# yehonatan145/PatternMatching

Hardware: AMD Instinct MI355X
Metric: GB/s stream scanned + matches/sec, snort.dict, 1/2/4/8 MI355X vs CPU ref (higher is better)
Workload: dtype u8

## Files before the change

### patternmatching_amd/csrc/pm_kernels.hip

```cpp
#include <type_traits>

#include <algorithm>

#include "pm_kernels.h"
#include "pm_streamgen.h"

namespace {

#ifdef RT_PLAIN_STORES
#define RT_OUT_STORE(v, p) (*(p) = (v))
#else
#define RT_OUT_STORE(v, p) __builtin_nontemporal_store((v), (p))
#endif
constexpr int RT_THREADS = 1024;
constexpr int RT_WAVES = RT_THREADS / 64;
constexpr int RT_T2_U16 = 65536;
constexpr int RT_FILTER_WORDS = 4096;
constexpr int RT_F3_WORDS = 256;
constexpr int RT_F2_WORDS = 2048;
constexpr uint32_t RT_QCAP = 64;
constexpr uint32_t RT_ROUND = 40;
constexpr int RT_CHUNK = 1024;
constexpr uint32_t CONT16 = 0x8000u;
constexpr uint32_t CONT32 = 0x80000000u;
constexpr uint32_t T3H_VALID = 1u << 24;
constexpr uint32_t RT_POSMASK = (1u << 30) - 1;
constexpr uint32_t RT_SLOT2 = 1u << 30;
constexpr uint32_t RT_REC_LEAF_K = 0, RT_REC_KIDS_K = 1, RT_REC_CHAIN_K = 2, RT_REC_WIDE_K = 3;

__device__ __forceinline__ uint32_t rt_hash(uint32_t k) { return k * 0x9E3779B1u; }
__device__ __forceinline__ uint32_t rt_fhash(uint32_t k) {
    uint32_t h;
    asm("v_mul_u32_u24 %0, 0x9e3779, %1" : "=v"(h) : "v"(k));
    return h;
}
__device__ __forceinline__ uint32_t rt_fhit(uint32_t w, uint32_t f) {
    uint32_t a, b, c;
    asm("v_lshrrev_b32_e32 %0, %1, %2" : "=v"(a) : "v"(f), "v"(w));
    asm("v_lshrrev_b32_sdwa %0, %1, %2 dst_sel:DWORD dst_unused:UNUSED_PAD src0_sel:BYTE_1 src1_sel:DWORD"
        : "=v"(b) : "v"(f), "v"(w));
    asm("v_lshrrev_b32_sdwa %0, %1, %2 dst_sel:DWORD dst_unused:UNUSED_PAD src0_sel:BYTE_2 src1_sel:DWORD"
        : "=v"(c) : "v"(f), "v"(w));
    return a & b & c & 1u;
}

struct Stage2 {
    uint32_t g3, g4, w3, w4;
};
__device__ __forceinline__ Stage2 rt_stage2_load(const uint32_t* s_f2, uint32_t q) {
    Stage2 z;
    asm("v_mul_u32_u24 %0, 0x85ebca, %1" : "=v"(z.g3) : "v"(q >> 8));
    z.g4 = q * 0x9E3779B1u;
    z.w3 = s_f2[z.g3 >> 24];
    z.w4 = s_f2[RT_F3_WORDS + (((z.g4 >> 20) * 7u) >> 4)];
    return z;
}
__device__ __forceinline__ uint32_t rt_stage2_hit(const Stage2& z) { return rt_fhit(z.w3, z.g3) | rt_fhit(z.w4, z.g4); }

__device__ __forceinline__ uint32_t wave_scan_incl(uint32_t x) {
    x += __builtin_amdgcn_update_dpp(0u, x, 0x111, 0xf, 0xf, false);
    x += __builtin_amdgcn_update_dpp(0u, x, 0x112, 0xf, 0xf, false);
    x += __builtin_amdgcn_update_dpp(0u, x, 0x114, 0xf, 0xf, false);
    x += __builtin_amdgcn_update_dpp(0u, x, 0x118, 0xf, 0xf, false);
    x += __builtin_amdgcn_update_dpp(0u, x, 0x142, 0xa, 0xf, false);
    x += __builtin_amdgcn_update_dpp(0u, x, 0x143, 0xc, 0xf, false);
    return x;
}

__device__ __forceinline__ uint32_t wave_prefix(uint64_t m) {
    return __builtin_amdgcn_mbcnt_hi((uint32_t)(m >> 32), __builtin_amdgcn_mbcnt_lo((uint32_t)m, 0u));
}

template <class V4>
__device__ __forceinline__ uint32_t rec_kind(const V4& R) { return R.x >> 30; }
template <class V4>
__device__ __forceinline__ uint32_t rec_kid_index(const V4& R, uint32_t c) {
    const uint32_t c4 = c * 0x01010101u;
    const uint32_t lo = R.z ^ c4, hi = R.w ^ c4;
    const uint32_t zl = (lo - 0x01010101u) & ~lo & 0x80808080u;
    const uint32_t zh = (hi - 0x01010101u) & ~hi & 0x80808080u;
    const uint32_t cnt = (R.x >> 24) & 63u;
    const uint32_t j = zl ? (uint32_t)__builtin_ctz(zl) >> 3 : zh ? 4u + ((uint32_t)__builtin_ctz(zh) >> 3) : 8u;
    return j < cnt ? j : cnt;
}

template <class V4>
__device__ __forceinline__ uint32_t wide_child(const V4& Q, uint32_t c) {
    const uint32_t odd = (c >> 5) & 1u, bit = c & 31u;
    const uint32_t word = odd ? Q.y : Q.x;
    if (!((word >> bit) & 1u)) return ~0u;
    return Q.z + (odd ? (uint32_t)__popc(Q.x) : 0u) + (uint32_t)__popc(word & ((1u << bit) - 1u));
}

template <bool FOLD>
__device__ __forceinline__ uint32_t rt_byte(const uint8_t* __restrict__ text, int64_t k) {
    uint32_t c = text[k];
    if (FOLD) c += c - 'A' < 26u ? 32u : 0u;
    return c;
}

template <bool FOLD = false>
__device__ __forceinline__ uint32_t rt_deep(const uint8_t* __restrict__ text, const RtDev& t, uint32_t node, int64_t i,
                                            int64_t avail, int64_t d) {
    for (;;) {
        const uint4 R = t.rec[node];
        if (d >= avail) return R.y;
        const uint32_t c = rt_byte<FOLD>(text, i - d);
        const uint32_t kind = rec_kind(R), first = R.x & 0xFFFFFFu;
        if (kind == RT_REC_LEAF_K) return R.y;
        if (kind == RT_REC_CHAIN_K) {
            const uint32_t L = (R.x >> 24) & 63u;
            const uint32_t lim = avail - d < (int64_t)L ? (uint32_t)(avail - d) : L;
            uint64_t win = 0;
#pragma unroll
            for (int k = 0; k < 8; ++k) {
                const uint32_t kk = (uint32_t)k < lim ? (uint32_t)k : lim - 1u;
                win |= (uint64_t)rt_byte<FOLD>(text, i - d - kk) << (8 * (7 - k));
            }
            const uint64_t dif = win ^ ((uint64_t)R.w << 32 | R.z);
            uint32_t m = dif ? (uint32_t)__builtin_clzll(dif) >> 3 : 8u;
            m = m < lim ? m : lim;
            if (m < L) return R.y;
            node = first + m - 1u;
            d += m;
            continue;
        } else if (kind == RT_REC_KIDS_K) {
            const uint32_t j = rec_kid_index(R, c);
            if (j == ((R.x >> 24) & 63u)) return R.y;
            node = first + j;
        } else {
            const uint32_t ch = wide_child(t.wide[(size_t)R.z * 4 + (c >> 6)], c);
            if (ch == ~0u) return R.y;
            node = ch;
        }
        ++d;
    }
}

__device__ __forceinline__ uint32_t rt_slot1(uint32_t k, uint32_t bits) { return rt_hash(k) >> (32 - bits); }
__device__ __forceinline__ uint32_t rt_slot2(uint32_t k, uint32_t bits) { return (k * 0x85EBCA77u) >> (32 - bits); }

template <bool FOLD = false>
__device__ __forceinline__ uint32_t rt_from_d2(const uint8_t* __restrict__ text, const RtDev& t, uint32_t key24,
                                               uint32_t c3, uint32_t best2, int64_t i, int64_t avail) {
    const uint32_t want = T3H_VALID | key24;
    uint4 e = t.t3h[rt_slot1(key24, t.t3h_bits)];
    if ((e.x & 0x1FFFFFFu) != want) {
        e = t.t3h[rt_slot2(key24, t.t3h_bits)];
        if ((e.x & 0x1FFFFFFu) != want) return best2;
    }
    const uint32_t kind = e.x >> 25;
    if (kind == 0 || avail < 4) return e.y;
    if (kind == 1) {
        const uint32_t nch = e.z >> 24;
        const uint32_t k = c3 == (e.z & 0xFFu) ? 0u : c3 == ((e.z >> 8) & 0xFFu) ? 1u : c3 == ((e.z >> 16) & 0xFFu) ? 2u : 3u;
        if (k >= nch) return e.y;
        if (nch > 1) return rt_deep<FOLD>(text, t, e.w + k, i, avail, 4);
        if (!(e.w & CONT32)) return e.w;
        return rt_deep<FOLD>(text, t, e.w & 0x7FFFFFFFu, i, avail, 4);
    }
    return rt_deep<FOLD>(text, t, e.w & 0x7FFFFFFFu, i, avail, 3);
}

template <bool FOLD = false>
__device__ uint32_t rt_one(const uint8_t* __restrict__ text, const uint16_t* s_t, const RtDev& t, int64_t i,
                           int64_t stream_start) {
    const int64_t avail = i - stream_start + 1;
    const uint32_t c0 = rt_byte<FOLD>(text, i);
    if (avail == 1) return t.t12[65536 + c0];
    const uint32_t c1 = rt_byte<FOLD>(text, i - 1);
    const uint32_t v = s_t[(c0 << 8) | c1];
    if (!(v & CONT16) || avail == 2) return v & 0x7FFFu;
    return rt_from_d2<FOLD>(text, t, rt_byte<FOLD>(text, i - 2) | (c1 << 8) | (c0 << 16),
                            avail >= 4 ? rt_byte<FOLD>(text, i - 3) : 0u, v & 0x7FFFu, i, avail);
}
// ... 118 lines not shown
            const uint64_t m = __ballot(need);
            const uint32_t idx = nxt + wave_prefix(m);
            if (need && idx < nwalk) {
                z.st = TS_ENTRY;
                z.c = idx & 1u;
                z.pa = reinterpret_cast<const tu32x4*>(items + (idx & ~1u));
                z.pb = dummy2;
            }
            nxt += (uint32_t)__popcll(m);
            if (nxt > nwalk) nxt = nwalk;
            busy |= z.st != TS_EMPTY;
        });
        if (!__ballot(busy)) break;
        unroll_for<0, SLOTS>([&](auto I) __attribute__((always_inline)) {
            TailSlot& z = S[I];
            z.A = *z.pa;
            z.B = *z.pb;
        });
        unroll_for<0, SLOTS>([&](auto I) __attribute__((always_inline)) {
            TailSlot& z = S[I];
            const uint32_t st = z.st;
            const tu32x4 A = z.A;
            const uint32_t en = z.c ? A.z : A.x, ep = z.c ? A.w : A.y;
            const uint32_t off = z.pos & RT_POSMASK;
            const int32_t rq = (int32_t)off - (int32_t)z.dd;
            const bool reload = rq < z.twa || rq >= z.twa + 8;
            const uint32_t rlo = reload ? z.B.x : z.tlo, rhi = reload ? z.B.y : z.thi;
            const int32_t rta = reload ? (rq & ~7) : z.twa;
            const uint32_t ro = (uint32_t)(rq - rta);
            const uint32_t c = ((ro & 4 ? rhi : rlo) >> (8 * (ro & 3))) & 0xFFu;
            const uint32_t rkind = rec_kind(A), first = A.x & 0xFFFFFFu;
            const uint32_t jr = rec_kid_index(A, c);
            const bool rend = z.dd >= z.av;
            const bool rnext = !rend && rkind == RT_REC_KIDS_K && jr != ((A.x >> 24) & 63u);
            const bool rwide = !rend && rkind == RT_REC_WIDE_K;
            const uint64_t win = ((uint64_t)rhi << 32 | rlo) << (8 * (7 - ro));
            const uint64_t dif = win ^ ((uint64_t)A.w << 32 | A.z);
            const uint32_t meq = dif ? (uint32_t)__builtin_clzll(dif) >> 3 : 8u;
            const uint32_t clen = (A.x >> 24) & 63u;
            const uint32_t cav = z.av > z.dd ? z.av - z.dd : 0u;
            const uint32_t clim = min(min(clen, ro + 1u), cav);
            const uint32_t cm = min(meq, clim);
            const bool cnext = rkind == RT_REC_CHAIN_K && cm >= 1u && (cm == clen || (cm == ro + 1u && cm < cav));
            const uint32_t wnode = wide_child(A, z.c);
            const bool wnext = wnode != ~0u;

            uint32_t nst = TS_EMPTY;
            bool fin = false;
            uint32_t ans = A.w;
            if (st == TS_ENTRY) {
                nst = TS_REC;
                z.node = en;
                z.dd = (ep & RT_D4) ? 4u : 3u;
                z.pos = ep & ~RT_D4;
                const uint32_t o = ep & RT_POSMASK;
                z.av = o + ctx + 1 > 1024u ? 1024u : o + ctx + 1;
                z.twa = INT32_MIN / 2;
            }
            if (st == TS_REC) {
                nst = (rnext || cnext) ? TS_REC : rwide ? TS_WIDE : TS_EMPTY;
                fin = !rnext && !rwide && !cnext;
                ans = A.y;
                z.tlo = rlo;
                z.thi = rhi;
                z.twa = rta;
                z.node = cnext ? first + cm - 1u : first + jr;
                z.dd += rnext ? 1u : cnext ? cm : 0u;
                z.c = c;
            }
            if (st == TS_WIDE) {
                nst = wnext ? TS_REC : TS_EMPTY;
                fin = !wnext;
                z.node = wnode;
                z.dd += 1;
            }
            if (fin) {
                cnt += (uint32_t)(ans != 0u) - (z.pos >> 31);
                if (OUTW) put_id<OUTW>(out, (int64_t)(z.pos & RT_POSMASK), ans);
            }
            z.st = nst;
            const int32_t nq = (int32_t)(z.pos & RT_POSMASK) - (int32_t)z.dd;
            const bool nreload = z.dd < z.av && (nq < z.twa || nq >= z.twa + 8);
            const tu32x4* pa = dummy4;
            const tu32x2* pb = dummy2;
            if (nst == TS_REC) {
                pa = RC + z.node;
                if (nreload) pb = reinterpret_cast<const tu32x2*>(tb + (nq & ~7));
            }
            if (nst == TS_WIDE) pa = WD + (size_t)A.z * 4 + (c >> 6);
            z.pa = pa;
            z.pb = pb;
        });
    }
    return nwalk;
}

template <int V, int OUTW, bool EF = false>
__global__ __launch_bounds__(RT_THREADS) void rt_scan_kernel(const uint8_t* __restrict__ text, int64_t stream_start,
                                                             int64_t pos0, int64_t n, void* __restrict__ out,
                                                             unsigned long long* __restrict__ count, RtDev t) {
    static_assert(V == 0 || V == 2, "product kernel (0) or streaming floor (2)");
    constexpr bool kT8 = V == 0 && OUTW == 0;
    constexpr int kLdsWords = kT8 ? RT_T2_U16 / 4 + RT_F2_WORDS + 2 * RT_WAVES * RT_QCAP
                                  : RT_FILTER_WORDS + RT_T2_U16 / 2 + RT_F2_WORDS + 2 * RT_WAVES * RT_QCAP;
    __shared__ __attribute__((aligned(16))) uint32_t s_lds[kLdsWords];
    uint32_t* const s_f = s_lds;
    const uint8_t* const s_t8 = reinterpret_cast<const uint8_t*>(s_lds);
    const uint16_t* const s_t = kT8 ? t.t12 : reinterpret_cast<uint16_t*>(s_lds + RT_FILTER_WORDS);
    uint32_t* const s_f2 = s_lds + (kT8 ? RT_T2_U16 / 4 : RT_FILTER_WORDS + RT_T2_U16 / 2);
    uint32_t(*const s_qkey)[RT_QCAP] = reinterpret_cast<uint32_t(*)[RT_QCAP]>(s_f2 + RT_F2_WORDS);
    uint32_t(*const s_qpos)[RT_QCAP] = s_qkey + RT_WAVES;
    {
        const uint4* fsrc = reinterpret_cast<const uint4*>(t.filt);
        if (kT8) {
            const uint2* src = reinterpret_cast<const uint2*>(t.t12);
            for (int k = threadIdx.x; k < RT_T2_U16 / 4; k += RT_THREADS) {
                const uint2 v = src[k];
                const uint32_t e[4] = {v.x & 0xFFFFu, v.x >> 16, v.y & 0xFFFFu, v.y >> 16};
                uint32_t w = 0;
#pragma unroll
                for (int q = 0; q < 4; ++q) {
                    const uint32_t nz = (e[q] & 0x7FFFu) != 0u, cand = !nz && (e[q] & CONT16);
                    w |= (nz | cand << 1) << (8 * q);
                }
                s_lds[k] = w;
            }
        } else {
            const uint4* src = reinterpret_cast<const uint4*>(t.t12);
            uint4* dst = reinterpret_cast<uint4*>(s_lds + RT_FILTER_WORDS);
            for (int k = threadIdx.x; k < RT_T2_U16 * 2 / 16; k += RT_THREADS) dst[k] = src[k];
            uint4* fdst = reinterpret_cast<uint4*>(s_f);
            for (int k = threadIdx.x; k < RT_FILTER_WORDS / 4; k += RT_THREADS) fdst[k] = fsrc[k];
        }
        uint4* f2dst = reinterpret_cast<uint4*>(s_f2);
        for (int k = threadIdx.x; k < RT_F2_WORDS / 4; k += RT_THREADS) f2dst[k] = fsrc[RT_FILTER_WORDS / 4 + k];
    }
    __syncthreads();

    constexpr bool kFilter = V == 0;
    constexpr bool kPushS2 = V == 0 && OUTW == 4;
    constexpr bool kRounds = !(V == 0 && OUTW == 0);
    constexpr bool kStage1 = !(V == 0 && OUTW == 0);
    const int lane = threadIdx.x & 63;
    const int wid = __builtin_amdgcn_readfirstlane(threadIdx.x >> 6);
    uint32_t* qkey = s_qkey[wid];
    uint32_t* qpos = s_qpos[wid];
    uint32_t cnt = 0;
    uint32_t scnt = 0;
    const int64_t nchunks = (n + RT_CHUNK - 1) / RT_CHUNK;
    const int64_t c_hi = n / RT_CHUNK;
    const int64_t c_lo = pos0 - stream_start >= 2 ? 0 : 1;
    const int64_t gw = (int64_t)blockIdx.x * RT_WAVES + wid;
    const int64_t nw = (int64_t)gridDim.x * RT_WAVES;
    const int64_t cbeg = c_lo + gw, cend = c_hi, cstep = nw;
    uint32_t* const sp = t.spill + 2 * gw * t.spill_stride;
    uint32_t sn = 0;
    const uint8_t* dummy = reinterpret_cast<const uint8_t*>(t.filt) + 4;
    using u32x2 = __attribute__((ext_vector_type(2))) unsigned int;
    using u32x4 = __attribute__((ext_vector_type(4))) unsigned int;

    struct Round {
        uint32_t n;
        uint32_t keep;
        uint32_t fk, fp;
        u32x2 tw;
        uint32_t skip;
        u32x4 L0;
    };
    uint32_t qh = 0, qn = 0;
    auto issue = [&](Round& r, uint32_t take) __attribute__((always_inline)) {
        __builtin_amdgcn_wave_barrier();
        const bool act = (uint32_t)lane < take;
        const uint32_t sl = (qh + lane) & (RT_QCAP - 1);
        r.fk = act ? qkey[sl] : 0u;
        r.fp = act ? qpos[sl] : 0u;
        const bool deep = r.fp >> 31;
        bool skip = false;
        if (!kPushS2 && take) {
            const bool first = act && !deep && !(r.fp & RT_SLOT2);
            if (first) skip = rt_stage2_hit(rt_stage2_load(s_f2, r.fk)) == 0u;
        }
        r.skip = skip;
        r.keep = (uint32_t)__popcll(__ballot(act && !skip));
        const uint32_t k = r.fk >> 8;
        const uint32_t node = r.fk & 0x7FFFFFu, d = r.fk >> 23;
        const bool wide = deep && (r.fp & RT_SLOT2);
        const int64_t i = pos0 + (int64_t)(r.fp & RT_POSMASK);
        const u32x4* T = reinterpret_cast<const u32x4*>(t.t3h);
        const u32x4* F = reinterpret_cast<const u32x4*>(t.filt);
        const uint32_t slot = (r.fp & RT_SLOT2) ? rt_slot2(k, t.t3h_bits) : rt_slot1(k, t.t3h_bits);
        const u32x4* W = reinterpret_cast<const u32x4*>(t.wide) + (size_t)(r.fk & 0x3FFFu) * 4 + ((r.fk >> 20) & 3u);
        const u32x4* a0 = wide ? W : deep ? reinterpret_cast<const u32x4*>(t.rec) + node : ((act && !skip) ? T + slot : F);
        const uint8_t* a1 = (deep && !wide && (int64_t)d <= i - stream_start) ? text + ((i - d) & ~(int64_t)7) : dummy;
        r.L0 = *a0;
        r.tw = *reinterpret_cast<const u32x2*>(a1);
        r.n = take;
        qh += take;
        qn -= take;
    };
    auto consume = [&](Round& r) __attribute__((always_inline)) {
        u32x4 L0 = r.L0;
        u32x2 tw = r.tw;
        uint32_t fk = r.fk, fp = r.fp;
        asm volatile("" : "+v"(L0), "+v"(tw), "+v"(fk), "+v"(fp)::"memory");
        bool again = false, wstep = false;
        uint32_t nk = 0, np = 0;
        if ((uint32_t)lane < r.n && !r.skip) {
            const int64_t i = pos0 + (int64_t)(fp & RT_POSMASK);
            const int64_t avail = i - stream_start + 1;
            uint32_t v, ph0 = 0xFFFFFFFFu, node = 0, d = 0;
            bool reprobe = false;
            if (!(fp >> 31)) {
                const uint32_t k = fk >> 8, c3 = fk & 0xFFu;
                ph0 = s_t[k >> 8] & 0x7FFFu;
                const uint32_t want = T3H_VALID | k;
                const u32x4 e = L0;
                v = ph0;
                if ((e.x & 0x1FFFFFFu) != want && (e.x & T3H_VALID) && !(fp & RT_SLOT2)) {
                    reprobe = true;
                    again = true;
                } else if ((e.x & 0x1FFFFFFu) == want) {
                    v = e.y;
                    const uint32_t kind = e.x >> 25;
                    if (avail >= 4 && kind == 1) {
                        const uint32_t nch = e.z >> 24;
                        const uint32_t j = c3 == (e.z & 0xFFu) ? 0u : c3 == ((e.z >> 8) & 0xFFu) ? 1u
                                         : c3 == ((e.z >> 16) & 0xFFu) ? 2u : 3u;
                        if (j < nch) {
                            if (nch == 1 && !(e.w & CONT32)) {
                                v = e.w;
                            } else {
                                again = true;
                                node = nch == 1 ? e.w & 0x7FFFFFFFu : e.w + j;
                                d = 4;
                            }
                        }
                    } else if (avail >= 4 && kind == 2) {
                        again = true;
                        node = e.w & 0x7FFFFFFFu;
                        d = 3;
                    }
                }
            } else if (fp & RT_SLOT2) {
                const uint32_t ch = wide_child(L0, (fk >> 14) & 0xFFu);
                d = (fk >> 22) + 1;
                v = L0.w;
                if (ch != ~0u) {
                    node = ch;
                    again = true;
                }
            } else {
                d = fk >> 23;
                const u32x4 R = L0;
                v = R.y;
                if ((int64_t)d < avail) {
                    const uint32_t kind = rec_kind(R);
                    const uint32_t ro = (uint32_t)(i - d) & 7u;
                    const uint32_t tc = (((ro & 4) ? tw.y : tw.x) >> (8 * (ro & 3))) & 0xFFu;
                    if (kind == RT_REC_CHAIN_K) {
                        const uint64_t win = ((uint64_t)tw.y << 32 | tw.x) << (8 * (7 - ro));
                        const uint64_t dif = win ^ ((uint64_t)R.w << 32 | R.z);
                        const uint32_t meq = dif ? (uint32_t)__builtin_clzll(dif) >> 3 : 8u;
                        const uint32_t clen = (R.x >> 24) & 63u;
                        const uint32_t cav = (uint32_t)(avail - d);
                        const uint32_t cm = min(meq, min(min(clen, ro + 1u), cav));
                        if (cm >= 1u && (cm == clen || (cm == ro + 1u && cm < cav))) {
                            node = (R.x & 0xFFFFFFu) + cm - 1u;
                            d += cm;
                            again = true;
                        }
                    } else if (kind == RT_REC_KIDS_K) {
                        const uint32_t j = rec_kid_index(R, tc);
                        if (j != ((R.x >> 24) & 63u)) {
                            node = (R.x & 0xFFFFFFu) + j;
                            ++d;
                            again = true;
                        }
                    } else if (kind == RT_REC_WIDE_K) {
                        wstep = true;
                        again = true;
                        node = R.z | (tc << 14);
                    }
                }
            }
            if (reprobe) {
                nk = fk;
                np = fp | RT_SLOT2;
            } else if (wstep) {
                nk = node | (d << 22);
                np = fp | RT_SLOT2;
            } else if (again) {
                nk = node | (d << 23);
                np = (fp & ~RT_SLOT2) | 0x80000000u;
                if (!(fp >> 31)) cnt -= (uint32_t)(ph0 != 0u);
            } else {
                cnt += (uint32_t)(v != 0u) - ((fp >> 31) ? 0u : (uint32_t)(ph0 != 0u));
                if (OUTW && v != ph0) put_id<OUTW>(out, i - pos0, v);
            }
        }
        __builtin_amdgcn_wave_barrier();
        const uint64_t m = __ballot(again);
        if (again) {
            const uint32_t sl = (qh + qn + wave_prefix(m)) & (RT_QCAP - 1);
            qkey[sl] = nk;
            qpos[sl] = np;
        }
        __builtin_amdgcn_wave_barrier();
        qn += (uint32_t)__popcll(m);
        r.n = 0;
        r.keep = 0;
    };
    auto fetch = [&](uint32_t (&xr)[4], uint32_t& xp, int64_t c) __attribute__((always_inline)) {
        const uint8_t* base = c < cend ? text + pos0 + c * RT_CHUNK : dummy;
#pragma unroll
        for (int s = 0; s < 4; ++s)
            xr[s] = __builtin_nontemporal_load(reinterpret_cast<const uint32_t*>(base + 256 * s + 4 * lane));
        xp = __builtin_nontemporal_load(reinterpret_cast<const uint32_t*>(base - 4));
    };
    auto stand_in_store = [&]() __attribute__((always_inline)) {
        if (OUTW == 4) {
            u32x4* o = reinterpret_cast<u32x4*>(t.scratch);
#pragma unroll
            for (int s = 0; s < 4; ++s) __builtin_nontemporal_store(u32x4{0u, 0u, 0u, 0u}, o + 64 * s + lane);
        }
        if (OUTW == 2) {
            u32x2* o = reinterpret_cast<u32x2*>(t.scratch);
#pragma unroll
            for (int s = 0; s < 4; ++s) __builtin_nontemporal_store(u32x2{0u, 0u}, o + 64 * s + lane);
        }
    };
    Round rr;
    rr.n = 0;
    rr.keep = 0;
    uint32_t xa[4], xb[4], pa, pb;
    int64_t ch = cbeg;
    const uint32_t scap = (uint32_t)t.spill_stride;
    auto resolve = [&]() __attribute__((always_inline)) {
        if (!kFilter) return;
        if (rr.n) consume(rr);
        while (qn) {
            Round rs;
            issue(rs, qn);
            consume(rs);
        }
        if (kRounds && t.spill_total && sn && lane == 0) atomicAdd(t.spill_total, (unsigned long long)sn);
        __builtin_amdgcn_s_waitcnt(0);
        {
            const uint32_t nwalk = rt_tail<OUTW>(text, stream_start, pos0, out, t, s_f2, sp, sn, lane, cnt);
            if (!kRounds && t.spill_total && nwalk && lane == 0)
                atomicAdd(t.spill_total, (unsigned long long)nwalk);
        }
        __builtin_amdgcn_s_waitcnt(0);
        sn = 0;
    };
    auto chunk = [&](uint32_t (&xr)[4], uint32_t& xp, int64_t c) __attribute__((always_inline)) {
        const int64_t pc = pos0 + c * RT_CHUNK;
        u32x2 x[4];
#pragma unroll
        for (int s = 0; s < 4; ++s) {
            const uint32_t fix = s == 0 ? xp : __builtin_amdgcn_update_dpp(0u, xr[s - 1], 0x13C, 0xf, 0xf, false);
            x[s].x = __builtin_amdgcn_update_dpp(fix, xr[s], 0x138, 0xf, 0xf, false);
            x[s].y = xr[s];
        }
        if (EF) fetch(xr, xp, c + 2 * cstep);
#define RT_RAW(j) ((uint32_t)((((uint64_t)x[(j) >> 2].y << 32) | x[(j) >> 2].x) >> (8 * (2 + ((j) & 3)))))
#define RT_KEY(j) (RT_RAW(j) & 0xFFFFFFu)
        uint32_t res[16];
        constexpr int CMS = kT8 ? 1 : 0;
        uint32_t cm = 0;
        if (kT8) {
            uint32_t f = 0;
            constexpr uint32_t kSel0 = 0x0C0C0000u;
#define RT_T8KEY(j) \
    __builtin_amdgcn_perm(x[(j) >> 2].y, x[(j) >> 2].x, kSel0 | (4u + ((j) & 3)) << 8 | (3u + ((j) & 3)))
#pragma unroll
            for (int j = 0; j < 16; ++j) f |= (uint32_t)s_t8[RT_T8KEY(j)] << (2 * j);
#undef RT_T8KEY
            cnt += (uint32_t)__popc(f & 0x55555555u);
            cm = f & 0xAAAAAAAAu;
        } else {
#pragma unroll
        for (int j = 0; j < 16; ++j) res[j] = V == 2 ? RT_KEY(j) & 0xFFFFu : s_t[RT_KEY(j) >> 8];
        if (kFilter && kStage1) {
            uint32_t fw[16];
#pragma unroll
            for (int j = 0; j < 16; ++j) fw[j] = s_f[rt_fhash(RT_RAW(j)) >> 20];
#pragma unroll
            for (int j = 0; j < 16; ++j) cm |= ((res[j] >> 15) & rt_fhit(fw[j], rt_fhash(RT_RAW(j)))) << j;
        } else if (kFilter) {
#pragma unroll
            for (int j = 0; j < 16; ++j) cm |= (res[j] >> 15) << j;
        }
        if (kFilter) {
            if (OUTW == 0) {
                uint32_t zm = 0;
#pragma unroll
                for (int j = 0; j < 16; ++j) zm |= (uint32_t)((res[j] & 0x7FFFu) == 0u) << j;
                cm &= zm;
            }
        }
#pragma unroll
        for (int j = 0; j < 16; ++j) {
            res[j] &= 0x7FFFu;
            scnt += (uint32_t)__popcll(__ballot(res[j] != 0u));
        }
        }
#undef RT_KEY
#undef RT_RAW
        if (kFilter && kRounds) {
            if (rr.n) consume(rr);
            issue(rr, qn >= RT_ROUND ? qn : 0u);
        }
        if (OUTW == 4) {
            u32x4* o = reinterpret_cast<u32x4*>(reinterpret_cast<uint32_t*>(out) + (pc - pos0));
#pragma unroll
            for (int s = 0; s < 4; ++s) {
                u32x4 v = {res[4 * s], res[4 * s + 1], res[4 * s + 2], res[4 * s + 3]};
                RT_OUT_STORE(v, o + 64 * s + lane);
            }
        }
        if (OUTW == 2) {
            u32x2* o = reinterpret_cast<u32x2*>(reinterpret_cast<uint16_t*>(out) + (pc - pos0));
#pragma unroll
            for (int s = 0; s < 4; ++s) {
                u32x2 v = {res[4 * s] | (res[4 * s + 1] << 16), res[4 * s + 2] | (res[4 * s + 3] << 16)};
                RT_OUT_STORE(v, o + 64 * s + lane);
            }
        }
        asm volatile("" ::: "memory");
        if (kPushS2) {
            uint32_t mm = cm, keep = 0;
            while (mm) {
                const uint32_t bit = __builtin_ctz(mm), j = bit >> CMS;
                mm &= mm - 1;
                const uint32_t sg = j >> 2, b = j & 3;
                const u32x2 w01 = (sg & 1) ? x[1] : x[0], w23 = (sg & 1) ? x[3] : x[2];
                const u32x2 w = (sg & 2) ? w23 : w01;
                const uint32_t q32 = (uint32_t)((((uint64_t)w.y << 32) | w.x) >> (8 * (1 + b)));
                keep |= (rt_stage2_hit(rt_stage2_load(s_f2, q32)) != 0u) << bit;
            }
            cm = keep;
        }
        if (kFilter) {
            const uint32_t c = __popc(cm);
            const uint32_t incl = wave_scan_incl(c);
            const uint32_t base = incl - c;
            const uint32_t total = __builtin_amdgcn_readlane(incl, 63);
            uint32_t mm = cm;
            const uint32_t pbase = (uint32_t)(pc - pos0) + 4 * lane;
            if (kRounds && total <= RT_QCAP - qn - rr.keep) {
                uint32_t slot = qh + qn + base;
                while (mm) {
                    const uint32_t j = __builtin_ctz(mm) >> CMS;
                    mm &= mm - 1;
                    const uint32_t sg = j >> 2, b = j & 3;
                    const u32x2 w01 = (sg & 1) ? x[1] : x[0], w23 = (sg & 1) ? x[3] : x[2];
                    const u32x2 w = (sg & 2) ? w23 : w01;
                    const uint32_t sl = slot & (RT_QCAP - 1);
                    qkey[sl] = (uint32_t)((((uint64_t)w.y << 32) | w.x) >> (8 * (1 + b)));
                    qpos[sl] = pbase + 256 * sg + b;
                    ++slot;
                }
                qn += total;
            } else {
                uint32_t room = kRounds ? RT_QCAP - qn - rr.keep : 0u;
                if (__builtin_expect(sn + (total - room) > scap, 0)) {
                    resolve();
                    room = kRounds ? min(RT_QCAP, total) : 0u;
                }
                uint32_t rank = base;
                while (mm) {
                    const uint32_t j = __builtin_ctz(mm) >> CMS;
                    mm &= mm - 1;
                    const uint32_t sg = j >> 2, b = j & 3;
                    const u32x2 w01 = (sg & 1) ? x[1] : x[0], w23 = (sg & 1) ? x[3] : x[2];
                    const u32x2 w = (sg & 2) ? w23 : w01;
                    const uint32_t q32 = (uint32_t)((((uint64_t)w.y << 32) | w.x) >> (8 * (1 + b)));
                    const uint32_t p = pbase + 256 * sg + b;
                    if (rank < room) {
                        const uint32_t sl = (qh + qn + rank) & (RT_QCAP - 1);
                        qkey[sl] = q32;
                        qpos[sl] = p;
                    } else {
                        const uint32_t ph = OUTW == 0 ? 0u : (uint32_t)((s_t[q32 >> 16] & 0x7FFFu) != 0u);
                        reinterpret_cast<u32x2*>(sp)[sn + rank - room] = u32x2{q32, p | (ph << 31)};
                    }
                    ++rank;
                }
                sn = __builtin_amdgcn_readfirstlane(sn + total - room);
                qn = __builtin_amdgcn_readfirstlane(qn + room);
            }
        }
        if (!EF) fetch(xr, xp, c + 2 * cstep);
    };
    Round r0;
    if (EF) fetch(xa, pa, ch);
    if (kFilter && kRounds) issue(r0, 0);
    stand_in_store();
    if (!EF) fetch(xa, pa, ch);
    if (EF) fetch(xb, pb, ch + cstep);
    if (kFilter && kRounds) issue(rr, 0);
    stand_in_store();
    if (!EF) fetch(xb, pb, ch + cstep);
    for (;;) {
        if (ch >= cend) break;
        chunk(xa, pa, ch);
        if (ch + cstep >= cend) break;
        chunk(xb, pb, ch + cstep);
        ch += 2 * cstep;
    }
    resolve();
    if (blockIdx.x == gridDim.x - 1) {
#pragma unroll 1
        for (int e = 0; e < 2; ++e) {
            int64_t c = -1;
            if (e == 0 && c_lo == 1) c = 0;
            if (e == 1 && c_hi < nchunks && !(c_lo == 1 && c_hi == 0)) c = c_hi;
            const int64_t p = pos0 + c * RT_CHUNK + threadIdx.x;
            if (c >= 0 && p < pos0 + n) {
                const uint32_t v = rt_one(text, s_t, t, p, stream_start);
                if (OUTW) put_id<OUTW>(out, p - pos0, v);
                cnt += v != 0u;
            }
        }
    }
    if (count) {
        for (int o = 32; o > 0; o >>= 1) cnt += __shfl_down(cnt, o);
        cnt += scnt;
        if (lane == 0 && cnt) atomicAdd(count, (unsigned long long)cnt);
    }
}

constexpr int RT_SMALL_THREADS = 256;
template <int OUTW>
__global__ __launch_bounds__(RT_SMALL_THREADS) void rt_small_kernel(const uint8_t* __restrict__ text,
                                                                    int64_t stream_start, int64_t pos0, int64_t n,
                                                                    void* __restrict__ out,
                                                                    unsigned long long* __restrict__ count, RtDev t) {
    const int64_t k = (int64_t)blockIdx.x * RT_SMALL_THREADS + threadIdx.x;
    uint32_t v = 0, deep = 0;
    if (k < n) {
        const int64_t i = pos0 + k;
        v = rt_one(text, t.t12, t, i, stream_start);
        if (t.spill_total && i - stream_start >= 3 && (t.t12[(uint32_t)text[i] << 8 | text[i - 1]] & CONT16)) {
            const uint32_t q = (uint32_t)text[i - 3] | (uint32_t)text[i - 2] << 8 | (uint32_t)text[i - 1] << 16 |
                               (uint32_t)text[i] << 24;
            const uint32_t f = rt_fhash(q >> 8);
            if (rt_fhit(t.filt[f >> 20], f)) deep = rt_stage2_hit(rt_stage2_load(t.filt + RT_FILTER_WORDS, q));
        }
        if (OUTW) put_id<OUTW>(out, k, v);
    }
    const uint64_t nz = __ballot(v != 0u), dp = __ballot(deep != 0u);
    if ((threadIdx.x & 63) == 0) {
        if (count && nz) atomicAdd(count, (unsigned long long)__popcll(nz));
        if (t.spill_total && dp) atomicAdd(t.spill_total, (unsigned long long)__popcll(dp));
    }
}

constexpr int RT_SERVE_WIN = 16384;
constexpr int RT_SERVE_POLLERS = 4;
#ifndef PM_SERVE_TRACE
#define PM_SERVE_TRACE 0
#endif
__device__ __forceinline__ uint64_t rfl64(uint64_t x) {
    const uint32_t lo = __builtin_amdgcn_readfirstlane((uint32_t)x);
    const uint32_t hi = __builtin_amdgcn_readfirstlane((uint32_t)(x >> 32));
    return (uint64_t)hi << 32 | lo;
}
__device__ __forceinline__ uint64_t lane64(uint64_t x, int l) {
    const uint32_t lo = __builtin_amdgcn_readlane((uint32_t)x, l);
    const uint32_t hi = __builtin_amdgcn_readlane((uint32_t)(x >> 32), l);
    return (uint64_t)hi << 32 | lo;
}
template <class T>
__device__ __forceinline__ T sys_load(const T* p) {
    return __hip_atomic_load(p, __ATOMIC_RELAXED, __HIP_MEMORY_SCOPE_SYSTEM);
}
template <class T>
__device__ __forceinline__ void sys_store(T* p, T v) {
    __hip_atomic_store(p, v, __ATOMIC_RELAXED, __HIP_MEMORY_SCOPE_SYSTEM);
}
template <class T>
__device__ __forceinline__ T dev_load(const T* p) {
    return __hip_atomic_load(p, __ATOMIC_RELAXED, __HIP_MEMORY_SCOPE_AGENT);
}
template <class T>
__device__ __forceinline__ void dev_store(T* p, T v) {
    __hip_atomic_store(p, v, __ATOMIC_RELAXED, __HIP_MEMORY_SCOPE_AGENT);
}
__global__ __launch_bounds__(RT_SERVE_THREADS) void rt_serve_kernel(PmServeReq* req, uint64_t* fwd, uint32_t* done,
                                                                    uint64_t seen, uint64_t gen, int64_t idle_ticks,
                                                                    RtDev t) {
    __shared__ __attribute__((aligned(16))) uint8_t win[RT_SERVE_WIN];
    __shared__ uint64_t s_w[8];
    __shared__ uint32_t s_state;
    const uint64_t* const rq = reinterpret_cast<const uint64_t*>(req);
    const int tid = threadIdx.x;
    const int wid = __builtin_amdgcn_readfirstlane(tid >> 6);
    const int64_t G = gridDim.x, wg = blockIdx.x;
    if (tid == 0) s_state = 0;
    __syncthreads();
    for (;;) {
        if (wg == 0 ? wid < RT_SERVE_POLLERS : wid == 0) {
            for (int q = 0; q < wid; ++q) __builtin_amdgcn_s_sleep(24);
            const uint64_t t0 = __builtin_amdgcn_s_memrealtime();
            uint64_t w = 0;
            uint32_t found = 0, quit = 0;
            const uint64_t* const src = wg == 0 ? rq : fwd;
            for (;;) {
                w = wg == 0 ? sys_load(src + (tid & 7)) : dev_load(src + (tid & 7));
                const uint64_t s2 = lane64(w, 7);
                if (s2 > seen && s2 == lane64(w, 0)) {
                    found = 1;
                    break;
                }
                if (lane64(w, 1) == gen || __builtin_amdgcn_s_memrealtime() - t0 > (uint64_t)idle_ticks) {
                    quit = 1;
                    break;
                }
                if (wg == 0 && __builtin_amdgcn_readfirstlane(
                                   __hip_atomic_load(&s_state, __ATOMIC_RELAXED, __HIP_MEMORY_SCOPE_WORKGROUP)))
                    break;
                __builtin_amdgcn_s_sleep(1);
            }
#if PM_SERVE_TRACE
            if ((tid & 63) == 0 && wg < 2 && found)
                sys_store(reinterpret_cast<uint64_t*>(done + G + 16) + 8 * wg, __builtin_amdgcn_s_memrealtime());
#endif
            if (found) {
                const int lane = tid & 63;
                uint32_t old = 1;
                if (lane == 0) old = __hip_atomic_exchange(&s_state, 1u, __ATOMIC_RELAXED, __HIP_MEMORY_SCOPE_WORKGROUP);
                if (__builtin_amdgcn_readfirstlane(old) != 1) {
                    if (lane < 8 && lane != 1) s_w[lane] = w;
                    if (wg == 0) {
                        if (lane >= 2 && lane < 7) dev_store(fwd + lane, w);
                        __builtin_amdgcn_s_waitcnt(0);
                        if (lane == 0 || lane == 7) dev_store(fwd + lane, w);
                    }
                }
            } else if (quit && (tid & 63) == 0) {
                uint32_t zero = 0;
                __hip_atomic_compare_exchange_strong(&s_state, &zero, 2u, __ATOMIC_RELAXED, __ATOMIC_RELAXED,
                                                     __HIP_MEMORY_SCOPE_WORKGROUP);
            }
        }
        __syncthreads();
        if (__builtin_amdgcn_readfirstlane(s_state) == 2) {
            if (wg == 0 && tid == 1) dev_store(fwd + 1, gen);
            return;
        }
        __syncthreads();
        if (tid == 0) s_state = 0;
        const uint64_t v = rfl64(s_w[0]);
        seen = v;
        const uint8_t* const text = reinterpret_cast<const uint8_t*>(rfl64(s_w[2]));
        void* const out = reinterpret_cast<void*>(rfl64(s_w[3]));
        const int64_t ss = (int64_t)rfl64(s_w[4]), pos0 = (int64_t)rfl64(s_w[5]);
        const uint64_t nw = rfl64(s_w[6]);
        const int64_t n = (int64_t)(nw & ((1ull << 56) - 1));
        const bool w4 = (nw >> 56) == 4;
        const int64_t per = ((n + G - 1) / G + 63) & ~(int64_t)63;
// ... 2462 lines not shown
        for (int off = 32; off > 0; off >>= 1) cnt += __shfl_down(cnt, off);
        if ((threadIdx.x & 63) == 0 && cnt) atomicAdd(count, (unsigned long long)cnt);
    }
}

__global__ __launch_bounds__(1024) void gather_probe_kernel(const uint32_t* __restrict__ tab, uint32_t words,
                                                            int steps, uint32_t* __restrict__ sink) {
    const uint32_t lane = blockIdx.x * 1024u + threadIdx.x;
    uint32_t idx = __umulhi(lane * 0x9E3779B1u, words), acc = 0;
    for (int j = 0; j < steps; ++j) {
        const uint32_t v = tab[idx];
        acc += v;
        idx = __umulhi((v ^ (lane + (uint32_t)j)) * 0x9E3779B1u, words);
    }
    if (acc == 0x9E3779B1u && idx == 1u) sink[0] = acc;
}

__device__ __forceinline__ void score_one(uint32_t a, uint32_t r, const uint32_t* __restrict__ parent,
                                          const uint32_t* __restrict__ depth, uint32_t (&c)[5]) {
    if (a == r) {
        ++c[0];
    } else if (a) {
        uint32_t cur = r;
        while (cur && cur != a) cur = parent[cur];
        ++c[cur ? 1 : 3];
    } else {
        ++c[2];
    }
    if (r) c[4] += depth[r];
}

constexpr int SCORE_THREADS = 256;

constexpr int SCORE_V = 2;
template <int V>
__global__ __launch_bounds__(SCORE_THREADS) void score_kernel(const uint32_t* __restrict__ algo,
                                                              const uint32_t* __restrict__ real, int64_t n,
                                                              const uint32_t* __restrict__ parent,
                                                              const uint32_t* __restrict__ depth,
                                                              unsigned long long* __restrict__ counts) {
    uint32_t c[5] = {0, 0, 0, 0, 0};
    const int64_t nv = n / 4;
    const int64_t stride = (int64_t)gridDim.x * SCORE_THREADS;
    using v4 = __attribute__((ext_vector_type(4))) unsigned int;
    const v4* A = reinterpret_cast<const v4*>(algo);
    const v4* R = reinterpret_cast<const v4*>(real);
    for (int64_t k = (int64_t)blockIdx.x * SCORE_THREADS + threadIdx.x; k < nv; k += V * stride) {
        v4 a[V], r[V];
#pragma unroll
        for (int j = 0; j < V; ++j) {
            const int64_t kj = k + j * stride;
            a[j] = kj < nv ? __builtin_nontemporal_load(A + kj) : v4{0, 0, 0, 0};
            r[j] = kj < nv ? __builtin_nontemporal_load(R + kj) : v4{0, 0, 0, 0};
        }
#pragma unroll
        for (int j = 0; j < V; ++j) {
            if (k + j * stride >= nv) break;
            score_one(a[j].x, r[j].x, parent, depth, c);
            score_one(a[j].y, r[j].y, parent, depth, c);
            score_one(a[j].z, r[j].z, parent, depth, c);
            score_one(a[j].w, r[j].w, parent, depth, c);
        }
    }
    if (blockIdx.x == 0 && threadIdx.x < (n & 3)) score_one(algo[4 * nv + threadIdx.x], real[4 * nv + threadIdx.x], parent, depth, c);
#pragma unroll
    for (int q = 0; q < 5; ++q) {
        unsigned long long v = c[q];
        for (int o = 32; o > 0; o >>= 1) v += __shfl_down(v, o);
        if ((threadIdx.x & 63) == 0 && v) atomicAdd(counts + q, v);
    }
}

constexpr int HIST_THREADS = 1024;
constexpr uint32_t HIST_WINDOW = 38912;
constexpr int HIST_V = 4;

template <int V>
__global__ __launch_bounds__(HIST_THREADS) void hist_kernel(const uint32_t* __restrict__ real, int64_t n,
                                                            const uint32_t* __restrict__ parent, uint32_t lo,
                                                            uint32_t cnt, unsigned long long* __restrict__ hist) {
    __shared__ uint32_t s_h[HIST_WINDOW];
    for (uint32_t k = threadIdx.x; k < cnt; k += HIST_THREADS) s_h[k] = 0;
    __syncthreads();
    using v4 = __attribute__((ext_vector_type(4))) unsigned int;
    const int64_t nv = n / 4;
    const int64_t stride = (int64_t)gridDim.x * HIST_THREADS;
    for (int64_t k = (int64_t)blockIdx.x * HIST_THREADS + threadIdx.x; k < nv; k += V * stride) {
        uint32_t g[4 * V];
#pragma unroll
        for (int j = 0; j < V; ++j) {
            const int64_t kj = k + j * stride;
            const v4 r = kj < nv ? __builtin_nontemporal_load(reinterpret_cast<const v4*>(real) + kj) : v4{0, 0, 0, 0};
            g[4 * j] = r.x;
            g[4 * j + 1] = r.y;
            g[4 * j + 2] = r.z;
            g[4 * j + 3] = r.w;
        }
        for (;;) {
            uint32_t any = 0;
#pragma unroll
            for (int i = 0; i < 4 * V; ++i) any |= g[i];
            if (!any) break;
#pragma unroll
            for (int i = 0; i < 4 * V; ++i)
                if (g[i] - lo < cnt) atomicAdd(&s_h[g[i] - lo], 1u);
#pragma unroll
            for (int i = 0; i < 4 * V; ++i) g[i] = g[i] ? parent[g[i]] : 0u;
        }
    }
    if (blockIdx.x == 0 && threadIdx.x < (n & 3)) {
        for (uint32_t g = real[4 * nv + threadIdx.x]; g; g = parent[g])
            if (g - lo < cnt) atomicAdd(&s_h[g - lo], 1u);
    }
    __syncthreads();
    for (uint32_t k = threadIdx.x; k < cnt; k += HIST_THREADS)
        if (s_h[k]) atomicAdd(hist + lo + k, (unsigned long long)s_h[k]);
}

__global__ void gen_lines_kernel(uint8_t* __restrict__ dst, uint64_t n, const uint8_t* __restrict__ pats,
                                 const uint32_t* __restrict__ offs, uint32_t npats, uint64_t seed) {
    const uint64_t nb = (n + PM_LINES_BLOCK - 1) / PM_LINES_BLOCK;
    const uint64_t stride = (uint64_t)gridDim.x * blockDim.x;
    for (uint64_t b = (uint64_t)blockIdx.x * blockDim.x + threadIdx.x; b < nb; b += stride) {
        const uint64_t lo = b * PM_LINES_BLOCK;
        pm_lines_block(dst + lo, n - lo < PM_LINES_BLOCK ? n - lo : PM_LINES_BLOCK, b, pats, offs, npats, seed);
    }
}

__global__ void gen_stream_kernel(uint8_t* __restrict__ dst, uint64_t off, uint64_t n, uint64_t seed, int mode) {
    const uint64_t stride = (uint64_t)gridDim.x * blockDim.x;
    for (uint64_t k = (uint64_t)blockIdx.x * blockDim.x + threadIdx.x; k < n; k += stride)
        dst[k] = pm_stream_byte(off + k, seed, mode);
}

}

static int64_t rt_blocks(int64_t n, int num_cu) {
    const int64_t nchunks = (n + RT_CHUNK - 1) / RT_CHUNK;
    const int64_t one_each = (nchunks + RT_WAVES - 1) / RT_WAVES;
    const int64_t eight_each = (nchunks + 8 * RT_WAVES - 1) / (8 * RT_WAVES);
    const int64_t floor_b = one_each < num_cu / 4 ? one_each : num_cu / 4;
    int64_t b = eight_each > floor_b ? eight_each : floor_b;
    if (b > num_cu) b = num_cu;
    return b < 1 ? 1 : b;
}
constexpr int64_t RT_SPILL_CAP_CHUNKS = 16;
constexpr int64_t RT_SPILL_FILL_COUNT = 4, RT_SPILL_FILL_IDS = 2;
static int64_t rt_wave_cap(int64_t cap_chunks, int outw = -1) {
    const int64_t dflt = outw < 0 ? RT_SPILL_CAP_CHUNKS : outw == 0 ? RT_SPILL_FILL_COUNT : RT_SPILL_FILL_IDS;
    return (cap_chunks >= 1 && cap_chunks < RT_SPILL_CAP_CHUNKS ? cap_chunks : dflt) * RT_CHUNK;
}
static int64_t rt_spill_stride(int64_t n, int64_t blocks, int64_t wave_cap) {
    const int64_t nw = blocks * RT_WAVES;
    const int64_t natural = ((n / RT_CHUNK + nw - 1) / nw) * RT_CHUNK;
    return natural < wave_cap ? natural : wave_cap;
}

hipError_t pm_launch_gather_probe(const uint32_t* table, uint32_t words, int steps, uint32_t* sink, int num_cu,
                                  hipStream_t s) {
    if (!table || words == 0 || steps <= 0 || num_cu <= 0) return hipErrorInvalidValue;
    hipLaunchKernelGGL(gather_probe_kernel, dim3((unsigned)num_cu), dim3(1024), 0, s, table, words, steps, sink);
    return hipGetLastError();
}

int64_t pm_rt_spill_items(int64_t n, int num_cu, int64_t cap_chunks) {
    constexpr int64_t PIECE = (int64_t)RT_POSMASK + 1;
    const int64_t m = n > PIECE ? PIECE : n;
    const int64_t blocks = rt_blocks(m, num_cu);
    return blocks * RT_WAVES * rt_spill_stride(m, blocks, rt_wave_cap(cap_chunks));
}

static hipError_t launch_rt_impl(bool floor, const uint8_t* text, int64_t stream_start, int64_t pos0, int64_t n,
                                 void* out, int outw, unsigned long long* count, const RtDev& t0, int num_cu,
                                 hipStream_t s) {
    if (n <= 0) return hipSuccess;
    if (!out) outw = 0;
    if (outw != 0 && outw != 2 && outw != 4) return hipErrorInvalidValue;
    constexpr int64_t PIECE = (int64_t)RT_POSMASK + 1;
    if (n > PIECE) {
        for (int64_t off = 0; off < n; off += PIECE) {
            const int64_t m = n - off < PIECE ? n - off : PIECE;
            void* o = outw ? reinterpret_cast<uint8_t*>(out) + off * outw : nullptr;
            hipError_t e = launch_rt_impl(floor, text, stream_start, pos0 + off, m, o, outw, count, t0, num_cu, s);
            if (e != hipSuccess) return e;
        }
        return hipSuccess;
    }
    const int64_t small_max = t0.small_max >= 0 ? t0.small_max : RT_SMALL_MAX;
    if (!floor && n <= small_max) {
        const dim3 gs((unsigned)((n + RT_SMALL_THREADS - 1) / RT_SMALL_THREADS)), bs(RT_SMALL_THREADS);
        if (outw == 4) hipLaunchKernelGGL((rt_small_kernel<4>), gs, bs, 0, s, text, stream_start, pos0, n, out, count, t0);
        else if (outw == 2) hipLaunchKernelGGL((rt_small_kernel<2>), gs, bs, 0, s, text, stream_start, pos0, n, out, count, t0);
        else hipLaunchKernelGGL((rt_small_kernel<0>), gs, bs, 0, s, text, stream_start, pos0, n, out, count, t0);
        return hipGetLastError();
    }
    const int64_t blocks = rt_blocks(n, num_cu);
    RtDev t = t0;
    t.spill_stride = rt_spill_stride(n, blocks, rt_wave_cap(t0.spill_cap_chunks, out ? outw : 0));
    const int64_t fit = t.spill_cap / (blocks * RT_WAVES) / RT_CHUNK * RT_CHUNK;
    if (t.spill_stride > fit) {
        if (fit < RT_CHUNK) return hipErrorInvalidValue;
        t.spill_stride = fit;
    }
    const dim3 g((unsigned)blocks), b(RT_THREADS);
    if (floor) {
        if (outw == 4) hipLaunchKernelGGL((rt_scan_kernel<2, 4>), g, b, 0, s, text, stream_start, pos0, n, out, count, t);
        else if (outw == 2) hipLaunchKernelGGL((rt_scan_kernel<2, 2>), g, b, 0, s, text, stream_start, pos0, n, out, count, t);
        else hipLaunchKernelGGL((rt_scan_kernel<2, 0>), g, b, 0, s, text, stream_start, pos0, n, out, count, t);
    } else if (outw == 4) {
        hipLaunchKernelGGL((rt_scan_kernel<0, 4>), g, b, 0, s, text, stream_start, pos0, n, out, count, t);
    } else if (outw == 2) {
        hipLaunchKernelGGL((rt_scan_kernel<0, 2, true>), g, b, 0, s, text, stream_start, pos0, n, out, count, t);
    } else {
        hipLaunchKernelGGL((rt_scan_kernel<0, 0, true>), g, b, 0, s, text, stream_start, pos0, n, out, count, t);
    }
    return hipGetLastError();
}

hipError_t pm_launch_rt(const uint8_t* text, int64_t stream_start, int64_t pos0, int64_t n, void* out, int outw,
                        unsigned long long* count, const RtDev& t, int num_cu, hipStream_t s) {
    return launch_rt_impl(false, text, stream_start, pos0, n, out, outw, count, t, num_cu, s);
}

static dim3 batch_grid(int64_t n, int64_t small_max, int num_cu, bool& small) {
    const int64_t ntiles = (n + RT_BATCH_TILE - 1) / RT_BATCH_TILE;
    small = n <= (small_max >= 0 ? small_max : RT_SMALL_MAX) && ntiles <= (int64_t)1 << 30;
    return dim3((unsigned)(small ? ntiles : ntiles < num_cu ? ntiles : num_cu));
}

static bool ev_ok(const EvDev& ev) { return ev.cursor && ev.len && ev.min_len >= 1 && (ev.events || !ev.cap); }

hipError_t pm_launch_rt_batch(const uint8_t* text, const int64_t* offsets, int64_t nseg, int64_t n, void* out,
                              int outw, unsigned long long* count, const RtDev& t, int num_cu, hipStream_t s) {
    if (n <= 0 || nseg <= 0) return hipSuccess;
    if (!text || !offsets || num_cu <= 0) return hipErrorInvalidValue;
    if (!out) outw = 0;
    if (outw != 0 && outw != 2 && outw != 4) return hipErrorInvalidValue;
    bool small;
    const dim3 g = batch_grid(n, t.small_max, num_cu, small), b(RT_THREADS);
#define PM_BATCH_LAUNCH(W_)                                                                                         \
    do {                                                                                                            \
        if (small) hipLaunchKernelGGL((rt_batch_kernel<W_, true>), g, b, 0, s, text, offsets, nseg, n, out, count, t); \
        else hipLaunchKernelGGL((rt_batch_kernel<W_, false>), g, b, 0, s, text, offsets, nseg, n, out, count, t);   \
    } while (0)
    if (outw == 4) PM_BATCH_LAUNCH(4);
    else if (outw == 2) PM_BATCH_LAUNCH(2);
    else PM_BATCH_LAUNCH(0);
#undef PM_BATCH_LAUNCH
    return hipGetLastError();
}

hipError_t pm_launch_rt_batch_events(const uint8_t* text, const int64_t* offsets, int64_t nseg, int64_t n,
                                     const EvDev& ev, const RtDev& t, int num_cu, hipStream_t s) {
    if (n <= 0 || nseg <= 0) return hipSuccess;
    if (!text || !offsets || num_cu <= 0 || !ev_ok(ev)) return hipErrorInvalidValue;
    bool small;
    const dim3 g = batch_grid(n, t.small_max, num_cu, small), b(RT_THREADS);
    if (small) hipLaunchKernelGGL(rt_batch_events_kernel<true>, g, b, 0, s, text, offsets, nseg, n, ev, t);
    else hipLaunchKernelGGL(rt_batch_events_kernel<false>, g, b, 0, s, text, offsets, nseg, n, ev, t);
    return hipGetLastError();
}

hipError_t pm_launch_rt_batch_matches(const uint8_t* text, const int64_t* offsets, int64_t nseg, int64_t n,
                                      const EvDev& ev, const MatchDev& mx, const RtDev& t, int num_cu, hipStream_t s) {
    if (n <= 0 || nseg <= 0) return hipSuccess;
    if (!text || !offsets || num_cu <= 0 || !ev_ok(ev) || !mx.parent) return hipErrorInvalidValue;
    bool small;
    const dim3 g = batch_grid(n, t.small_max, num_cu, small), b(RT_THREADS);
    if (small) hipLaunchKernelGGL(rt_batch_matches_kernel<true>, g, b, 0, s, text, offsets, nseg, n, ev, mx, t);
    else hipLaunchKernelGGL(rt_batch_matches_kernel<false>, g, b, 0, s, text, offsets, nseg, n, ev, mx, t);
    return hipGetLastError();
}

hipError_t pm_launch_rt_batch_groups(const uint8_t* text, const int64_t* offsets, int64_t nseg, int64_t n,
                                     const EvDev& ev, const MatchDev& mx, const GroupDev& gr, bool all,
                                     const RtDev& t, int num_cu, hipStream_t s) {
    if (n <= 0 || nseg <= 0) return hipSuccess;
    if (!text || !offsets || num_cu <= 0 || !ev_ok(ev) || !mx.parent || !gr.gmask || !gr.reach)
        return hipErrorInvalidValue;
    bool small;
    const dim3 g = batch_grid(n, t.small_max, num_cu, small), b(RT_THREADS);
    auto* const k = small ? (all ? rt_batch_groups_kernel<true, true> : rt_batch_groups_kernel<true, false>)
                          : (all ? rt_batch_groups_kernel<false, true> : rt_batch_groups_kernel<false, false>);
    hipLaunchKernelGGL(k, g, b, 0, s, text, offsets, nseg, n, ev, mx, gr, t);
    return hipGetLastError();
}

hipError_t pm_launch_rt_batch_windows(const uint8_t* text, const int64_t* offsets, int64_t nseg, int64_t n,
                                      const EvDev& ev, const MatchDev& mx, const GroupDev& gr, const WinDev& wn,
                                      bool all, const RtDev& t, int num_cu, hipStream_t s) {
    if (n <= 0 || nseg <= 0) return hipSuccess;
    if (!text || !offsets || num_cu <= 0 || !ev_ok(ev) || !mx.parent || !wn.win || !gr.gmask != !gr.reach ||
        (!gr.gmask && gr.stream_groups))
        return hipErrorInvalidValue;
    bool small;
    const dim3 g = batch_grid(n, t.small_max, num_cu, small), b(RT_THREADS);
    auto* const k = small ? (all ? rt_batch_windows_kernel<true, true> : rt_batch_windows_kernel<true, false>)
                          : (all ? rt_batch_windows_kernel<false, true> : rt_batch_windows_kernel<false, false>);
    hipLaunchKernelGGL(k, g, b, 0, s, text, offsets, nseg, n, ev, mx, gr, wn, t);
    return hipGetLastError();
}

hipError_t pm_launch_rt_serve(PmServeReq* req, uint64_t* fwd, uint32_t* done, int blocks, uint64_t seen,
                              uint64_t gen, int64_t idle_ticks, const RtDev& t, hipStream_t s) {
    if (blocks <= 0) return hipErrorInvalidValue;
    hipLaunchKernelGGL(rt_serve_kernel, dim3((unsigned)blocks), dim3(RT_SERVE_THREADS), 0, s, req, fwd, done, seen,
                       gen, idle_ticks, t);
// ... 347 lines not shown
```

Before: 920.9.

## Assign contiguous chunk-pair runs per wave and carry boundary bytes across chunks

Waves now scan contiguous tiles of two adjacent chunks, grouped into runs of RT_RUN tiles when OUTW is 4, instead of interleaving single chunks with stride nw. The 4-byte lookback for the second chunk and for later tiles within a run comes from a DPP carry of the previous chunk's last word rather than a separate global load. This gives more sequential memory access and fewer lookback loads. The spill stride sizing is recomputed from the new split, and uneven remainder handling adds index arithmetic and some risk of load imbalance.

```diff
diff --git a/patternmatching_amd/csrc/pm_kernels.hip b/patternmatching_amd/csrc/pm_kernels.hip
--- a/patternmatching_amd/csrc/pm_kernels.hip
+++ b/patternmatching_amd/csrc/pm_kernels.hip
@@ -21,6 +21,16 @@
 constexpr uint32_t RT_QCAP = 64;
 constexpr uint32_t RT_ROUND = 40;
 constexpr int RT_CHUNK = 1024;
+constexpr int RT_RUN = 4;
+struct RtSplit {
+    uint32_t kfull;
+    uint32_t q, s;
+};
+__host__ __device__ inline RtSplit rt_split(int64_t fast_chunks, int64_t nw, int run) {
+    const uint32_t tiles = (uint32_t)((fast_chunks + 1) / 2), round = (uint32_t)(run * nw);
+    const uint32_t kfull = tiles / round, rem = tiles - kfull * round;
+    return RtSplit{kfull, rem / (uint32_t)nw, rem % (uint32_t)nw};
+}
 constexpr uint32_t CONT16 = 0x8000u;
 constexpr uint32_t CONT32 = 0x80000000u;
 constexpr uint32_t T3H_VALID = 1u << 24;
@@ -445,7 +455,27 @@
     const int64_t c_lo = pos0 - stream_start >= 2 ? 0 : 1;
     const int64_t gw = (int64_t)blockIdx.x * RT_WAVES + wid;
     const int64_t nw = (int64_t)gridDim.x * RT_WAVES;
-    const int64_t cbeg = c_lo + gw, cend = c_hi, cstep = nw;
+    const int64_t cend = c_hi;
+    constexpr int kRun = OUTW == 4 ? RT_RUN : 1;
+    const RtSplit split = rt_split(c_hi - c_lo, nw, kRun);
+    auto run_at = [&](uint32_t k, int64_t& a0, int& len) __attribute__((always_inline)) {
+        const uint32_t g = (uint32_t)gw;
+        if (k < split.kfull) {
+            a0 = c_lo + 2 * (int64_t)((k * (uint32_t)nw + g) * kRun);
+            len = kRun;
+        } else {
+            const uint32_t l = k == split.kfull ? split.q + (g < split.s) : 0u;
+            a0 = l ? c_lo + 2 * (int64_t)(split.kfull * (uint32_t)nw * kRun + g * split.q + min(g, split.s)) : cend;
+            len = (l && kRun > 1) ? (int)l : 1;
+        }
+    };
+    uint32_t rk = 0;
+    int64_t cbeg, nbeg;
+    int run, nrun;
+    run_at(0, cbeg, run);
+    run_at(1, nbeg, nrun);
+    int ri = 0;
+    auto next_a = [&](int64_t c) __attribute__((always_inline)) { return ri + 1 < run ? c + 2 : nbeg; };
     uint32_t* const sp = t.spill + 2 * gw * t.spill_stride;
     uint32_t sn = 0;
     const uint8_t* dummy = reinterpret_cast<const uint8_t*>(t.filt) + 4;
@@ -603,12 +633,12 @@
         r.n = 0;
         r.keep = 0;
     };
-    auto fetch = [&](uint32_t (&xr)[4], uint32_t& xp, int64_t c) __attribute__((always_inline)) {
+    auto fetch = [&](uint32_t (&xr)[4], uint32_t& xp, int64_t c, bool kB, bool lb) __attribute__((always_inline)) {
         const uint8_t* base = c < cend ? text + pos0 + c * RT_CHUNK : dummy;
 #pragma unroll
         for (int s = 0; s < 4; ++s)
             xr[s] = __builtin_nontemporal_load(reinterpret_cast<const uint32_t*>(base + 256 * s + 4 * lane));
-        xp = __builtin_nontemporal_load(reinterpret_cast<const uint32_t*>(base - 4));
+        if (!kB) xp = __builtin_nontemporal_load(reinterpret_cast<const uint32_t*>((lb ? base : dummy) - 4));
     };
     auto stand_in_store = [&]() __attribute__((always_inline)) {
         if (OUTW == 4) {
@@ -625,7 +655,8 @@
     Round rr;
     rr.n = 0;
     rr.keep = 0;
-    uint32_t xa[4], xb[4], pa, pb;
+    uint32_t xa[4], xb[4], pa, none = 0;
+    uint32_t carry = 0;
     int64_t ch = cbeg;
     const uint32_t scap = (uint32_t)t.spill_stride;
     auto resolve = [&]() __attribute__((always_inline)) {
@@ -646,16 +677,20 @@
         __builtin_amdgcn_s_waitcnt(0);
         sn = 0;
     };
-    auto chunk = [&](uint32_t (&xr)[4], uint32_t& xp, int64_t c) __attribute__((always_inline)) {
+    auto chunk = [&](uint32_t (&xr)[4], uint32_t& xp, int64_t c, bool kB) __attribute__((always_inline)) {
         const int64_t pc = pos0 + c * RT_CHUNK;
         u32x2 x[4];
+        const uint32_t back = (kB || ri) ? carry : xp;
 #pragma unroll
         for (int s = 0; s < 4; ++s) {
-            const uint32_t fix = s == 0 ? xp : __builtin_amdgcn_update_dpp(0u, xr[s - 1], 0x13C, 0xf, 0xf, false);
+            const uint32_t fix = s == 0 ? back : __builtin_amdgcn_update_dpp(0u, xr[s - 1], 0x13C, 0xf, 0xf, false);
             x[s].x = __builtin_amdgcn_update_dpp(fix, xr[s], 0x138, 0xf, 0xf, false);
             x[s].y = xr[s];
         }
-        if (EF) fetch(xr, xp, c + 2 * cstep);
+        carry = __builtin_amdgcn_update_dpp(0u, xr[3], 0x13C, 0xf, 0xf, false);
+        const int64_t cn = kB ? next_a(c - 1) + 1 : next_a(c);
+        const bool lbn = ri + 1 >= run;
+        if (EF) fetch(xr, xp, cn, kB, lbn);
 #define RT_RAW(j) ((uint32_t)((((uint64_t)x[(j) >> 2].y << 32) | x[(j) >> 2].x) >> (8 * (2 + ((j) & 3)))))
 #define RT_KEY(j) (RT_RAW(j) & 0xFFFFFFu)
         uint32_t res[16];
@@ -784,23 +819,28 @@
                 qn = __builtin_amdgcn_readfirstlane(qn + room);
             }
         }
-        if (!EF) fetch(xr, xp, c + 2 * cstep);
+        if (!EF) fetch(xr, xp, cn, kB, lbn);
     };
     Round r0;
-    if (EF) fetch(xa, pa, ch);
+    if (EF) fetch(xa, pa, ch, false, true);
     if (kFilter && kRounds) issue(r0, 0);
     stand_in_store();
-    if (!EF) fetch(xa, pa, ch);
-    if (EF) fetch(xb, pb, ch + cstep);
+    if (!EF) fetch(xa, pa, ch, false, true);
+    if (EF) fetch(xb, none, ch + 1, true, false);
     if (kFilter && kRounds) issue(rr, 0);
     stand_in_store();
-    if (!EF) fetch(xb, pb, ch + cstep);
+    if (!EF) fetch(xb, none, ch + 1, true, false);
     for (;;) {
         if (ch >= cend) break;
-        chunk(xa, pa, ch);
-        if (ch + cstep >= cend) break;
-        chunk(xb, pb, ch + cstep);
-        ch += 2 * cstep;
+        chunk(xa, pa, ch, false);
+        if (ch + 1 >= cend) break;
+        chunk(xb, none, ch + 1, true);
+        ch = next_a(ch);
+        if (++ri >= run) {
+            ri = 0;
+            run = nrun;
+            run_at(++rk + 1, nbeg, nrun);
+        }
     }
     resolve();
     if (blockIdx.x == gridDim.x - 1) {
@@ -3569,7 +3609,9 @@
 }
 static int64_t rt_spill_stride(int64_t n, int64_t blocks, int64_t wave_cap) {
     const int64_t nw = blocks * RT_WAVES;
-    const int64_t natural = ((n / RT_CHUNK + nw - 1) / nw) * RT_CHUNK;
+    const RtSplit sp = rt_split(n / RT_CHUNK, nw, RT_RUN), s1 = rt_split(n / RT_CHUNK, nw, 1);
+    const int64_t runs = (int64_t)sp.kfull * RT_RUN + sp.q + (sp.s ? 1 : 0), ones = (int64_t)s1.kfull + (s1.s ? 1 : 0);
+    const int64_t natural = 2 * (runs > ones ? runs : ones) * RT_CHUNK;
     return natural < wave_cap ? natural : wave_cap;
 }
 
```

Measured after the change: 938.8 (median of 6 runs). +1.9%, better.
